# wsakobe/CylinderTag

Measured on AMD Instinct MI355X. Metric: frames/sec detect() 1920x1080, higher is better.
Workload: dtype u8; 1 GPU; synthetic 1920x1080 random-stripe frames, 4096 per step over 1 GPU(s), 4 planted CTag_2f12c markers each, detect(img,5,true,5), inputs resident in HBM; frames_per_gpu=4096, chunk=4096, parallelism=frames sharded, dp1, gather=none (1 GPU)

## Files before the change

cylindertag_amd/csrc/ctag_api.hip:

```cpp
#include <hip/hip_runtime.h>

#include <algorithm>
#include <climits>
#include <cmath>
#include <cstdio>
#include <cstdlib>
#include <cstring>
#include <fstream>
#include <map>
#include <mutex>
#include <new>
#include <string>
#include <type_traits>
#include <vector>

#include "../../include/ctag.h"
#include "ctag_internal.h"

using namespace ctag;

#define HIP_TRY(expr)                                                                                   \
    do {                                                                                                \
        hipError_t e__ = (expr);                                                                        \
        if (e__ != hipSuccess) {                                                                        \
// ... 123 lines not shown
    struct {
        void* p = nullptr;
        void (*free_fn)(void*) = nullptr;
    } state[kNumSiblingStates];
};

namespace ctag {
void** handle_state_slot(ctag_handle* h, SiblingState which, void (*free_fn)(void*)) {
    h->state[which].free_fn = free_fn;
    return &h->state[which].p;
}
bool handle_timing(const ctag_handle* h) { return h->timing; }
int handle_device(const ctag_handle* h) { return h->device; }
int handle_dict_cols(const ctag_handle* h) { return h->dict_cols; }
void handle_view(const ctag_handle* h, HandleView* out) {
    out->device = h->device;
    out->ws = h->last_ws && h->last_ws->base ? h->last_ws : nullptr;
    out->last_chunk_frames = h->last_chunk_frames;
    out->keep_pre = h->keep_pre;
    out->dict = h->dict.data();
    out->dict_rows = h->dict_rows;
    out->dict_cols = h->dict_cols;
    out->fused = h->last_plan.fused;
    out->frames = h->last_frames;
    out->row_stride = h->last_row_stride;
    out->frame_stride = h->last_frame_stride;
    out->stream = h->stream;
    out->gray = h->last_was_bgr ? h->d_gray.p : nullptr;
    out->gray_row_stride = h->gray_row_stride;
    out->gray_frame_stride = h->gray_frame_stride;
}
}

static const char* kStageNames[CTAG_NUM_STAGES] = {"decimate",  "threshold_ccl", "seam_merge", "resolve", "candidates", "quad_pack", "quad_edges", "quad_edges_big",
                                                    "line_sort", "welsch",        "quad_final", "features", "edge_refine", "markers"};

static FrameGeom make_geom(int rows, int cols, int tw, double area_max_fraction = 0.01) {
    FrameGeom g{};
    g.rows = rows;
    g.cols = cols;
    g.hrows = rows / 2;
    g.hcols = cols / 2;
    g.hp = (g.hcols + 63) & ~63;
    g.lp = (g.hcols + 63) & ~63;
    g.tw = tw;
    g.trows = g.hrows / tw + (g.hrows % tw != 0 ? 1 : 0);
// ... 96 lines not shown
    put(W.ymax, pool);
    put(W.key, pool);
    put(W.pool_tile, pool);
    put(W.member_head, pool);
    put(W.member_next, pool);
    put(W.ncand, F * 4);
    put(W.nroots, F * 4);
    put(W.cand, F * CC * sizeof(Candidate));
    put(W.quads, F * CC * sizeof(QuadOut));
    put(W.line_count, F * 4);
    put(W.clp_used, F * 4);
    put(W.line_long, F * 4);
    put(W.cl_pool, F * (size_t)W.cl_cap * 4 + 16);
    put(W.line_desc, F * LC * sizeof(LineDesc));
    put(W.line_sorted, F * LC * 4);
    put(W.line_fit, F * LC * 16);
    put(W.cand_aux, F * CC * sizeof(CandAux));
    put(W.npacks, F * 8);
    put(W.packs, F * CC * 4);
    put(W.pack_order, F * CC * 4);
    put(W.npacks2, F * 8);
    put(W.packs2, F * CC * 4);
    put(W.pack_order2, F * CC * 4);
    put(W.welsch_rs, std::min<size_t>(F, kLatencyFrames) * kLatLines * 20 * 6 * 4);
    put(W.quad_derived, F * kQuadStride * 48);
    put(W.quad_index, F * kQuadStride * 4);
    put(W.nquads, F * 4);
    put(W.nfeat, F * 4);
    put(W.status, F * 4);
    put(W.feat0, F * CTAG_MAX_FEATURES * sizeof(FeatureDev));
    put(W.feat1, F * CTAG_MAX_FEATURES * sizeof(FeatureDev));
    put(W.feat2, F * CTAG_MAX_FEATURES * sizeof(FeatureDev));
    put(W.premarkers, F * sizeof(ctag_frame_result));
    put(W.frame_long, F * 4);
    put(W.rz_xofs, (size_t)g.hcols * 4);
    put(W.rz_alpha, (size_t)g.hcols * 8);
    put(W.rz_yofs, (size_t)g.hrows * 4);
    put(W.rz_beta, (size_t)g.hrows * 8);
    return off;
}

static int ensure_workspace(ctag_handle* h, ctag_handle::WsSlot& S, int rows, int cols, int tw, int frames, bool big, bool need_n0) {
    auto refresh = [&](Workspace& W) {
        const Caps c = make_caps(make_geom(rows, cols, tw, h->params.area_max_fraction), h->params, big);
        W.g = make_geom(rows, cols, tw, h->params.area_max_fraction);
        W.g.pool_cap = c.pool_cap;
// ... 1025 lines not shown
```

cylindertag_amd/csrc/ctag_internal.h:

```cpp
#pragma once
#include <hip/hip_runtime.h>
#include <stddef.h>
#include <stdint.h>

#include <vector>

#include "../../include/ctag_types.h"

struct ctag_handle;
struct ctag_camera;
struct ctag_pose_rec;
struct ctag_rig_pose_rec;
struct ctag_mv_pose_rec;
struct ctag_camera_set;

namespace ctag {
template <class T>
struct DevBuf {
    T* p = nullptr;
    size_t cap = 0;
    DevBuf() = default;
    DevBuf(const DevBuf&) = delete;
    DevBuf& operator=(const DevBuf&) = delete;
    ~DevBuf() { release(); }
// ... 155 lines not shown
    int32_t* member_next = nullptr;
    int32_t* ncand = nullptr;
    int32_t* nroots = nullptr;
    int cand_cap = 0;
    int line_cap = 0;
    uint32_t cl_cap = 0;
    bool big = false;
    Candidate* cand = nullptr;
    QuadOut* quads = nullptr;
    int32_t* line_count = nullptr;
    int32_t* clp_used = nullptr;
    uint32_t* cl_pool = nullptr;
    LineDesc* line_desc = nullptr;
    int32_t* line_sorted = nullptr;
    int32_t* line_long = nullptr;
    float* line_fit = nullptr;
    CandAux* cand_aux = nullptr;
    int32_t* npacks = nullptr;
    uint32_t* packs = nullptr;
    uint32_t* pack_order = nullptr;
    int32_t* npacks2 = nullptr;
    uint32_t* packs2 = nullptr;
    uint32_t* pack_order2 = nullptr;
    float* welsch_rs = nullptr;
    const uint8_t* pick_table = nullptr;
    const uint16_t* pick_table16 = nullptr;
    hipStream_t aux_stream = nullptr;
    hipEvent_t ev_fork = nullptr, ev_join = nullptr;
    KParams kp{};
    void* quad_derived = nullptr;
    int32_t* quad_index = nullptr;
    int32_t* nquads = nullptr;
    int32_t* nfeat = nullptr;
    int32_t* status = nullptr;
    FeatureDev* feat0 = nullptr;
    FeatureDev* feat1 = nullptr;
    FeatureDev* feat2 = nullptr;
    ctag_frame_result* premarkers = nullptr;
    double* refine_n0 = nullptr;
    int32_t* frame_long = nullptr;
    int32_t* rz_xofs = nullptr;
    int16_t* rz_alpha = nullptr;
    int32_t* rz_yofs = nullptr;
    int16_t* rz_beta = nullptr;
    void* base = nullptr;
    size_t bytes = 0;
// ... 104 lines not shown
void build_pick_table(uint8_t* table, uint16_t* table16);


enum SiblingState { kPoseState, kDrawState, kRigState, kGatherState, kMvState, kCovState, kFitState, kRigFitState, kCamFitState, kIntrFitState, kNumSiblingStates };
void** handle_state_slot(struct ::ctag_handle* h, SiblingState which, void (*free_fn)(void*));
int model_to_device(struct ::ctag_model* m, int device);
int rigs_to_device(struct ::ctag_rigs* r, int device);
bool camera_ok(const struct ::ctag_camera* c);
bool handle_timing(const struct ::ctag_handle* h);
int handle_finish_pending(struct ::ctag_handle* h);
bool handle_pending_state(struct ::ctag_handle* h, const int32_t** count_dev, uint64_t* gen);
void handle_pending_clean(struct ::ctag_handle* h, uint64_t gen);
int handle_device(const struct ::ctag_handle* h);
int handle_dict_cols(const struct ::ctag_handle* h);

struct HandleView {
    int device;
    const Workspace* ws;
    int last_chunk_frames;
    bool keep_pre;
    const int32_t* dict;
    int dict_rows, dict_cols;
    bool fused;
    const uint8_t* frames;
    ptrdiff_t row_stride, frame_stride;
    hipStream_t stream;
    const uint8_t* gray;
    ptrdiff_t gray_row_stride, gray_frame_stride;
};
void handle_view(const struct ::ctag_handle* h, HandleView* out);
int mfit_probe_system(struct ::ctag_handle* h, const ctag_frame_result* results, int n_frames, const struct ::ctag_pose_rec* poses, int n_poses,
                      const struct ::ctag_model* model, const struct ::ctag_camera* camera, int model_index, double lambda, int min_obs, int pass_records,
                      double* S, double* g, double* delta, int32_t* held, int32_t* bad_pivot);
int mfit_record_grid();
int mfit_pass_records();
int rfit_probe_system(struct ::ctag_handle* h, const ctag_frame_result* results, int n_frames, const struct ::ctag_rig_pose_rec* recs,
                      const struct ::ctag_model* model, const struct ::ctag_rigs* rigs, const struct ::ctag_camera* camera, int rig, double lambda,
                      int pass_records, double* S, double* g, double* delta, int32_t* n_unknowns, int32_t* bad_pivot);
int cfit_probe_system(struct ::ctag_handle* h, const ctag_frame_result* results, int n_frames, const struct ::ctag_mv_pose_rec* recs,
                      const struct ::ctag_model* model, const struct ::ctag_rigs* rigs, const struct ::ctag_camera_set* cams, int anchor, double lambda,
                      int pass_records, double* S, double* g, double* delta, int32_t* n_unknowns, int32_t* bad_pivot);
int ifit_probe_system(struct ::ctag_handle* h, const ctag_frame_result* results, int n_frames, const struct ::ctag_rig_pose_rec* recs,
                      const struct ::ctag_model* model, const struct ::ctag_rigs* rigs, const struct ::ctag_camera* camera, uint32_t free_mask, int tie_focal,
                      double lambda, int pass_records, double* S, double* g, double* delta, int32_t* n_free, int32_t* bad_pivot);
int ifit_probe_poses(struct ::ctag_handle* h, const ctag_frame_result* results, int n_frames, const struct ::ctag_rig_pose_rec* recs,
                     const struct ::ctag_model* model, const struct ::ctag_rigs* rigs, const struct ::ctag_camera* camera, struct ::ctag_rig_pose_rec* out,
// ... 11 lines not shown
```

cylindertag_amd/csrc/k_quad.hip:

```cpp
#include "ctag_internal.h"
#include "ctag_math.h"
#include "ctag_wave.h"
#include <cstdio>
#include <type_traits>
#include <cstdlib>

namespace ctag {

struct QuadPtrs {
    const uint16_t* labels;
    const int32_t* tile_base;
    const int32_t* root_of;
    const int32_t* ncand;
    const Candidate* cand;
    QuadOut* quads;
    uint32_t* frame_flags;
    int32_t* line_count;
    int32_t* clp_used;
    uint32_t* cl_pool;
    LineDesc* line_desc;
    int32_t* line_sorted;
    int32_t* line_long;
    float* line_fit;
    CandAux* cand_aux;
    const uint8_t* pick_table;
    const uint16_t* pick_table16;
    const int32_t* pool_tile;
    const int32_t* member_head;
    const int32_t* member_next;
    int32_t* npacks;
    uint32_t* packs;
    uint32_t* pack_order;
    int32_t* npacks2;
    uint32_t* packs2;
    uint32_t* pack_order2;
    unsigned long long* stamps;
    float thr_line, thr_expand, rac;
    int c2_far, c2_near;
    int cand_cap, line_cap;
    uint32_t cl_cap;
    float expand_eps;
    const uint64_t* mask;
    int mask_words;
};
static QuadPtrs quad_ptrs(const ChunkPlan& pl, const Workspace& ws, unsigned long long* stamps) {
    QuadPtrs P{};
    P.labels = ws.labels, P.tile_base = ws.tile_base, P.root_of = ws.root_of, P.ncand = ws.ncand, P.cand = ws.cand, P.quads = ws.quads, P.frame_flags = ws.frame_flags;
    P.line_count = ws.line_count, P.clp_used = ws.clp_used, P.cl_pool = ws.cl_pool, P.line_desc = ws.line_desc, P.line_sorted = ws.line_sorted, P.line_long = ws.line_long;
    P.line_fit = ws.line_fit, P.cand_aux = ws.cand_aux, P.pick_table = ws.pick_table, P.pick_table16 = ws.pick_table16;
    P.pool_tile = ws.pool_tile, P.member_head = ws.member_head, P.member_next = ws.member_next;
    P.npacks = ws.npacks, P.packs = ws.packs, P.pack_order = ws.pack_order, P.stamps = stamps;
    P.npacks2 = ws.npacks2, P.packs2 = ws.packs2, P.pack_order2 = ws.pack_order2;
    P.thr_line = ws.kp.thr_line, P.thr_expand = ws.kp.thr_expand, P.rac = ws.kp.rac, P.c2_far = ws.kp.c2_far, P.c2_near = ws.kp.c2_near, P.expand_eps = ws.kp.expand_eps;
    P.cand_cap = ws.cand_cap, P.line_cap = ws.line_cap, P.cl_cap = ws.cl_cap;
    P.mask = pl.fused ? reinterpret_cast<const uint64_t*>(ws.half) : nullptr, P.mask_words = ws.g.hcols >> 6;
    return P;
}

__device__ __forceinline__ uint32_t pack_xy(int x, int y) { return (uint32_t)x | ((uint32_t)y << 16); }
__device__ __forceinline__ int ux(uint32_t p) { return (int)(p & 0xffffu); }
__device__ __forceinline__ int uy(uint32_t p) { return (int)(p >> 16); }

__device__ __forceinline__ void moments_to_line(double x, double y, double x2, double y2, double xy, double w, float* line) {
    const ctm::Recip64 W = ctm::recip64(w);
    x = ctm::div64(x, W);
    y = ctm::div64(y, W);
    x2 = ctm::div64(x2, W);
    y2 = ctm::div64(y2, W);
    xy = ctm::div64(xy, W);
    const double dx2 = x2 - x * x, dy2 = y2 - y * y, dxy = xy - x * y;
    const float t = (float)ctm::atan2_64(2 * dxy, dx2 - dy2) / 2;
    double sn, cs;
    ctm::sincos64(t, &sn, &cs);
    line[0] = (float)cs;
    line[1] = (float)sn;
// ... 218 lines not shown
    restart_store(res, rstride, line, err);
}

#ifndef CTAG_PACK_WORDS
#define CTAG_PACK_WORDS 5120
#endif
#ifndef CTAG_PACK_WAVES
#define CTAG_PACK_WAVES 2
#endif
constexpr int kPackWords = CTAG_PACK_WORDS;
#ifndef CTAG_PACK_WAVES_P2
#define CTAG_PACK_WAVES_P2 4
#endif
constexpr int kPackWordsSmall = 2560, kPackWavesSmall = 4, kPackWavesSmallP2 = CTAG_PACK_WAVES_P2;
constexpr int kUnwind = 8;
constexpr int kWaveWords = 8192;
constexpr int kWaveWordsMax = 36864;
__host__ __device__ __forceinline__ int pack_points(int w, int h) { return min(2 * (w + h), w * h) + 1; }
__host__ __device__ __forceinline__ int pack_need(int w, int h) {
    const int C = pack_points(w, h);
    return ((w + 1) & ~1) + 2 * h + 2 * C + 4;
}
__host__ __device__ __forceinline__ int need2(int n) { return 2 * ((n + 1) & ~1); }
constexpr int kScanWords = 2048;
__host__ __device__ __forceinline__ int scan_need(int w, int h) { return w + 3 * h + 4; }
constexpr int kMaskScanWords = 512, kMaskScanWordsLarge = 2048;
__host__ __device__ __forceinline__ int mask_scan_need(int w, int h) { return h * ((w + 31) / 32 + 1); }
__host__ __device__ __forceinline__ bool pack_big(int x_min, int w, int h, int big_points, int pack_words, int scan_words = 0) {
    (void)x_min;
    return pack_need(w, h) > pack_words || pack_points(w, h) > big_points || (scan_words > 0 && scan_need(w, h) > scan_words) ||
           (scan_words < 0 && mask_scan_need(w, h) > -scan_words);
}

struct CornerPre {
    float x, y, dis, ang;
};

__device__ __forceinline__ int pack_rank_sort(const int* s_key, uint16_t* s_ord, int n, int tid, int nt) {
    int neg = 0;
    for (int i = tid; i < n; i += nt) {
        const int ki = s_key[i];
        int rank = 0;
        for (int j = 0; j < n; j++) {
            const int kj = s_key[j];
            rank += (kj > ki || (kj == ki && j < i)) ? 1 : 0;
        }
// ... 137 lines not shown
    uint32_t* order2 = P.pack_order2 + (size_t)frame * P.cand_cap;
    uint32_t* packs2 = P.packs2 + (size_t)frame * P.cand_cap;
    auto key_of = [&](int r) {
        const CandAux a = aux[order[r]];
        return (a.line0 >= 0 && a.n_boundary > 0) ? a.n_boundary : -1;
    };
    int nel, np;
    if (npk > kLdsCand) {
        nel = pack_counting_sort(s_key, order2, npk, tid, nt, key_of, [&](int r) { return order[r]; });
        np = build_packs(packs2, nel, max_per_pack, pack_words, tid, [&](int r) { return need2(aux[order2[r]].n_boundary); });
    } else {
        for (int r = tid; r < npk; r += nt) s_key[r] = key_of(r);
        if (tid == 0) s_key[kLdsCand] = 0;
        __syncthreads();
        if (const int neg = pack_rank_sort(s_key, s_ord, npk, tid, nt)) atomicAdd(&s_key[kLdsCand], neg);
        __syncthreads();
        nel = npk - s_key[kLdsCand];
        for (int i = tid; i < nel; i += nt) order2[i] = order[s_ord[i]];
        np = build_packs(packs2, nel, max_per_pack, pack_words, tid, [&](int r) { return need2(s_key[s_ord[r]]); });
    }
    if (tid == 0) {
        P.npacks2[2 * frame] = np;
        P.npacks2[2 * frame + 1] = nel;
    }
}


#ifndef CTAG_EXPAND_INLINE
#define CTAG_EXPAND_INLINE __forceinline__
#endif
struct ALine {
    double c, s, x, y;
    bool ok;
};
__device__ __forceinline__ ALine approx_line(long long sx, long long sy, long long sxx, long long syy, long long sxy, int cnt, double k2lim) {
    const double n = (double)cnt, fx = (double)sx, fy = (double)sy;
    const double rn = __builtin_amdgcn_rcp(n);
    const double A = ((double)sxx * n - fx * fx) - ((double)syy * n - fy * fy);
    const double B = 2.0 * ((double)sxy * n - fx * fy);
    const double h2 = A * A + B * B;
    const double rh = __builtin_amdgcn_rsq(h2);
    const double u = ctm::fabs64(A) * rh;
    const double p = 0.5 + 0.5 * u;
    const double rp = __builtin_amdgcn_rsq(p);
    const double big = p * rp, small = (0.5 * ctm::fabs64(B) * rh) * rp;
    const bool bneg = B < 0.0;
// ... 368 lines not shown
                aux->line0 = p0;
                aux->acx = 0.f;
                aux->acy = 0.f;
                aux->n_boundary = 0;
            }
        }
    }
}

template <int SG, int WORDS, int WAVES, bool DYN, bool REFPRM, int PHASE = 0, bool PRESCAN = false>
__global__ __launch_bounds__(64) __attribute__((amdgpu_waves_per_eu(WAVES, WAVES))) void k_quad_edges_packed(QuadPtrs P, FrameGeom g, int nframes, int tier_lo) {
    static_assert(PHASE != 3 || (SG == 64 && !PRESCAN), "the scan-only build is a whole-wave build");
    static_assert(!PRESCAN || (SG == 8 && PHASE != 2), "PRESCAN: a packed build that would otherwise scan");
    const float k_thr_line = REFPRM ? 1.8f : P.thr_line, k_thr_expand = REFPRM ? 1.2f : P.thr_expand;
    const int k_c2_far = REFPRM ? 2 : P.c2_far, k_c2_near = REFPRM ? 1 : P.c2_near;
    static_assert(SG == 8 || SG == 64, "8 lanes per component (packs) or the whole wave (oversize components)");
    __shared__ uint32_t s_static[DYN ? 1 : WORDS];
    extern __shared__ uint32_t s_dynamic[];
    uint32_t* const s_mem = DYN ? s_dynamic : s_static;
    const int frame = blockIdx.x;
    if (frame >= nframes) return;
    const int lane = threadIdx.x, sub = lane / SG, sl = lane % SG, lane0 = lane - sl;
    const int nc = min(P.ncand[frame], P.cand_cap);
    const int npk = PHASE == 3 ? nc - P.npacks[2 * frame + 1]
                  : PHASE == 2 ? P.npacks2[2 * frame]
                               : P.npacks[2 * frame + (SG == 8 ? 0 : 1)];
    static_assert(PHASE != 2 || SG == 8, "the second kernel is a packed build");
    const uint32_t* __restrict__ pack_list = (PHASE == 2 ? P.packs2 : P.packs) + (size_t)frame * P.cand_cap;
    const uint32_t* __restrict__ pack_ord = (PHASE == 2 ? P.pack_order2 : P.pack_order) + (size_t)frame * P.cand_cap;
    const uint16_t* __restrict__ limg = P.labels + ((size_t)frame * g.hrows) * g.lp;
    const int32_t* __restrict__ tbase = P.tile_base + (size_t)frame * g.tiles_x * g.tiles_y;
    const int32_t* __restrict__ rootof = P.root_of + (size_t)frame * g.pool_cap;

    unsigned long long t_prev = 0;
    auto stamp = [&](int phase) {
        if (P.stamps) {
            const unsigned long long t = __builtin_amdgcn_s_memtime();
            if (phase >= 0 && lane == 0) atomicAdd(&P.stamps[phase + (SG == 64 ? 8 : 0)], t - t_prev);
            t_prev = t;
        }
    };
    for (int pk = blockIdx.y; pk < npk; pk += gridDim.y) {
        __syncthreads();
        stamp(-1);
        int first, cnt;
        if constexpr (SG == 8) {
            const uint32_t pw = pack_list[pk];
            first = (int)(pw & 0xffffffu);
            cnt = (int)(pw >> 24);
        } else if constexpr (PHASE == 3) {
            first = pk;
            cnt = 1;
        } else {
            first = nc - npk + pk;
            cnt = 1;
        }
        const bool act = sub < cnt;
        const int ci = (int)pack_ord[first + (act ? sub : 0)];
        const Candidate cd = P.cand[(size_t)frame * P.cand_cap + ci];
        CandAux* aux = P.cand_aux + (size_t)frame * P.cand_cap + ci;
        const int x_min = cd.x_min, y_min = cd.y_min;
        const int w = cd.x_max - cd.x_min + 1, h = cd.y_max - cd.y_min + 1;
        const int C = pack_points(w, h);
        int nb2 = 0;
        if constexpr (PHASE == 2) nb2 = aux->n_boundary;
        const int need = act ? (PHASE == 3 ? scan_need(w, h) : PHASE == 2 ? need2(nb2) : pack_need(w, h)) : 0;
        int off = 0;
#pragma unroll
        for (int k = 0; k < 64 / SG; k++) {
            const int v = __shfl(need, k * SG);
            if (k < sub) off += v;
        }
        if (!act) continue;
        if constexpr (SG == 64 && PHASE != 3) {
            if (need <= tier_lo) continue;
            if (need > WORDS) {
                if (tier_lo > 0 && sl == 0) {
                    atomicOr(&P.frame_flags[frame], CTAG_FLAG_POOL_OVERFLOW);
                    aux->line0 = -1;
                    aux->acx = 0.f;
                    aux->acy = 0.f;
                    aux->n_boundary = 0;
                }
                continue;
            }
        }
        uint32_t* mem = s_mem + off;
        uint32_t* tb = mem;
        uint32_t* lr = tb + w + 2;
        uint32_t* bufA = PHASE == 2 ? mem + (need >> 1) : lr + h + 2;
        uint32_t* bufB = PHASE == 2 ? mem : bufA + (PHASE == 3 ? h : C);
        uint32_t* lef = bufA;
        uint32_t* rig = bufB;
        const int sgshift = sub * SG;

        int n = 0, n_boundary = 0, p0 = 0;
        float acx = 0.f, acy = 0.f;
        if constexpr (PHASE != 2 && !PRESCAN) {
        stamp(6);
#ifndef CTAG_KEYS_LARGE
#define CTAG_KEYS_LARGE 16
#endif
#ifndef CTAG_KEYS_SMALL
#define CTAG_KEYS_SMALL 8
#endif
        constexpr int kMaxKeys = (SG == 8 && WORDS > kPackWordsSmall) ? CTAG_KEYS_LARGE : CTAG_KEYS_SMALL;
        uint32_t mykey[kMaxKeys];
        bool many = false;
        {
            const int32_t* ptile = P.pool_tile + (size_t)frame * g.pool_cap;
            const int32_t* mnext = P.member_next + (size_t)frame * g.pool_cap;
            int e = cd.root;
            bool first_e = true;
#pragma unroll
// ... 482 lines not shown
                }
                continue;
            }
            uint32_t* slot = P.cl_pool + (size_t)frame * P.cl_cap + p0;
            for (int x = sl; x < w + 2; x += SG) slot[x] = tb[x];
            for (int y = sl; y < h + 2; y += SG) slot[w + 2 + y] = lr[y];
            if (sl == 0) {
                aux->line0 = p0;
                aux->acx = 0.f;
                aux->acy = 0.f;
                aux->n_boundary = 0;
            }
            continue;
        }
        if constexpr (PHASE != 2) {
        if constexpr (PRESCAN) {
            p0 = aux->line0;
            if (p0 < 0) continue;
            const uint32_t* slot = P.cl_pool + (size_t)frame * P.cl_cap + p0;
            for (int x = sl; x < w + 2; x += SG) tb[x] = slot[x];
            for (int y = sl; y < h + 2; y += SG) lr[y] = slot[w + 2 + y];
            wave_fence();
        }
        int ntotal = 0;
        for (int x = sl; x < w; x += SG) {
            const uint32_t t = tb[x + 1];
            if (t) ntotal += 1 + ((t & 0xffffu) != (t >> 16) ? 1 : 0);
        }
        for (int y = sl; y < h; y += SG) {
            const uint32_t v = lr[y + 1];
            if (v) {
                const uint32_t ky = (uint32_t)(y + 2), xl = (v & 0xffffu) - 2u, xr = (v >> 16) - 2u;
                const uint32_t tl = tb[xl + 1], tr = tb[xr + 1];
                if ((tl & 0xffffu) != ky && (tl >> 16) != ky) ntotal++;
                if (xr != xl && (tr & 0xffffu) != ky && (tr >> 16) != ky) ntotal++;
            }
        }
        ntotal = sg_sum<SG>(ntotal);
        stamp(0);
        n = 0;
        {
            const int jd = sl & 7;
            const int dxl = (int)((0x01A9u >> (2 * jd)) & 3u) - 1, dyl = (int)((0x1A90u >> (2 * jd)) & 3u) - 1;
            int sp = 0;
            int fx = 0, fy = 0, j0 = 0;
            {
                const uint32_t c0 = tb[1];
                if (c0 == 0u) {
                    sp = -1;
                } else {
                    fy = (int)(c0 & 0xffffu) - 2;
                    n = 1;
                }
            }
            wave_fence();
            if (sp >= 0 && sl == 0) {
                bufA[0] = pack_xy(x_min, fy + y_min);
                uint32_t c = tb[1];
                if ((c >> 16) == (uint32_t)(fy + 2)) c &= 0xffffu;
                c &= 0xffff0000u;
                tb[1] = c;
// ... 66 lines not shown
                        }
                    }
                }
            } else {
                while (sp >= 0 && n < ntotal) {
                    const int nx = fx + dxl, ny = fy + dyl;
                    const uint32_t c = tb[nx + 1], r = lr[ny + 1];
                    const uint32_t ky = (uint32_t)(ny + 2), kx = (uint32_t)(nx + 2);
                    const bool hit = sl < 8 && sl >= j0 && ((c & 0xffffu) == ky || (c >> 16) == ky || (r & 0xffffu) == kx || (r >> 16) == kx);
                    const unsigned m = (unsigned)((__ballot(hit) >> sgshift) & 0xffull);
                    if (!m) {
                        sp--;
                        if (sp >= 0) {
                            const uint32_t f = bufB[sp];
                            fx = (int)(f & 0x3fff);
                            fy = (int)((f >> 14) & 0x3fff);
                            j0 = (int)(f >> 28);
                        }
                        continue;
                    }
                    const int j = __ffs(m) - 1;
                    const int hx = fx + ((int)((0x01A9u >> (2 * j)) & 3u) - 1), hy = fy + ((int)((0x1A90u >> (2 * j)) & 3u) - 1);
                    if (sl == j) {
                        if (n < C) bufA[n] = pack_xy(hx + x_min, hy + y_min);
                        uint32_t c2 = c, r2 = r;
                        if ((c2 & 0xffffu) == ky) c2 &= 0xffff0000u;
                        if ((c2 >> 16) == ky) c2 &= 0xffffu;
                        if ((r2 & 0xffffu) == kx) r2 &= 0xffff0000u;
                        if ((r2 >> 16) == kx) r2 &= 0xffffu;
                        tb[nx + 1] = c2;
                        lr[ny + 1] = r2;
                        if (sp <= C) bufB[sp] = (uint32_t)hx | ((uint32_t)hy << 14) | ((uint32_t)(j + 1) << 28);
                    }
                    wave_fence();
                    n++;
                    fx = hx;
                    fy = hy;
                    if (sp + 1 <= C) {
                        sp++;
                        j0 = 0;
                    } else {
                        j0 = j + 1;
                    }
                }
            }
            n = min(n, C);
        }
        n_boundary = n;
        if (n == 0) {
            if (sl == 0) {
                aux->line0 = -1;
                aux->acx = 0.f;
                aux->acy = 0.f;
                aux->n_boundary = 0;
            }
            continue;
        }
        wave_fence();
        stamp(1);
        {
            unsigned long long sx = 0, sy = 0;
            for (int k = sl; k < n; k += SG) {
                sx += (unsigned)ux(bufA[k]);
                sy += (unsigned)uy(bufA[k]);
            }
            sx = (unsigned long long)sg_sum<SG>((long long)sx);
            sy = (unsigned long long)sg_sum<SG>((long long)sy);
            acx = (float)(1.0 * (long long)sx / (double)(unsigned long long)n);
            acy = (float)(1.0 * (long long)sy / (double)(unsigned long long)n);
// ... 879 lines not shown
    out->valid = valid;
#pragma unroll
    for (int j = 0; j < 4; j++) {
        out->c[2 * j] = valid ? bc[j].x : 0.f;
        out->c[2 * j + 1] = valid ? bc[j].y : 0.f;
    }
}

#ifndef CTAG_SCAN_WAVES
#define CTAG_SCAN_WAVES 4
#endif
template <bool REF>
static void launch_quad_edges(const ChunkPlan& pl, const QuadPtrs& P, const FrameGeom& g, hipStream_t s, hipStream_t sb, hipStream_t s_max, hipEvent_t mid) {
    const int nframes = pl.nframes;
    const dim3 grid(nframes, pl.pack_gx);
    if (pl.all_wave) {
    } else if (pl.prescan) {
        if (pl.mask_scan)
            if (pl.small_cfg) hipLaunchKernelGGL((k_silhouette_mask<4, 32, kMaskScanWords>), dim3(nframes, pl.mscan_gx), dim3(64), 0, s, P, g, nframes);
            else hipLaunchKernelGGL((k_silhouette_mask<8, 64, kMaskScanWordsLarge>), dim3(nframes, 2 * pl.mscan_gx), dim3(64), 0, s, P, g, nframes);
        else
            hipLaunchKernelGGL((k_quad_edges_packed<64, kScanWords, CTAG_SCAN_WAVES, false, true, 3>), dim3(nframes, pl.scan_gx), dim3(64), 0, s, P, g, nframes, 0);
        if (pl.small_cfg) {
            hipLaunchKernelGGL((k_quad_edges_packed<8, kPackWordsSmall, kPackWavesSmall, false, REF, 1, true>), grid, dim3(64), 0, s, P, g, nframes, 0);
            hipLaunchKernelGGL(k_repack, dim3(nframes), dim3(64), 0, s, P, nframes, pl.pack_max, kPackWordsSmall);
            hipLaunchKernelGGL((k_quad_edges_packed<8, kPackWordsSmall, kPackWavesSmallP2, false, REF, 2>), grid, dim3(64), 0, s, P, g, nframes, 0);
        } else {
            hipLaunchKernelGGL((k_quad_edges_packed<8, kPackWords, CTAG_PACK_WAVES, false, REF, 0, true>), grid, dim3(64), 0, s, P, g, nframes, 0);
        }
    } else if (pl.small_cfg) {
        hipLaunchKernelGGL((k_quad_edges_packed<8, kPackWordsSmall, kPackWavesSmall, false, REF, 1>), grid, dim3(64), 0, s, P, g, nframes, 0);
        hipLaunchKernelGGL(k_repack, dim3(nframes), dim3(64), 0, s, P, nframes, pl.pack_max, kPackWordsSmall);
        hipLaunchKernelGGL((k_quad_edges_packed<8, kPackWordsSmall, kPackWavesSmallP2, false, REF, 2>), grid, dim3(64), 0, s, P, g, nframes, 0);
    } else {
        hipLaunchKernelGGL((k_quad_edges_packed<8, kPackWords, CTAG_PACK_WAVES, false, REF>), grid, dim3(64), 0, s, P, g, nframes, 0);
    }
    if (mid) (void)hipEventRecord(mid, s);
    ensure_dynamic_lds(reinterpret_cast<const void*>(&k_quad_edges_packed<64, kWaveWordsMax, 1, true, REF>), kWaveWordsMax * 4);
    hipLaunchKernelGGL((k_quad_edges_packed<64, kWaveWords, 1, false, REF>), dim3(nframes, pl.big_cols), dim3(64), 0, sb, P, g, nframes, 0);
    hipLaunchKernelGGL((k_quad_edges_packed<64, kWaveWordsMax, 1, true, REF>), dim3(nframes, pl.big_max_gx), dim3(64), kWaveWordsMax * 4, s_max, P, g, nframes, kWaveWords);
}

hipError_t launch_line_fits(const ChunkPlan& pl, const Workspace& ws, hipStream_t s, unsigned long long* stamps, hipEvent_t ev_sorted) {
    const int nframes = pl.nframes;
    const QuadPtrs P = quad_ptrs(pl, ws, stamps);
    hipLaunchKernelGGL(k_line_sort, dim3(nframes), dim3(kLineSortThreads), 0, s, P, nframes);
// ... 105 lines not shown
```

include/ctag_testkit.h:

```cpp
#ifndef CTAG_TESTKIT_H
#define CTAG_TESTKIT_H
#include <stddef.h>
#include <stdint.h>

#include "ctag.h"
#include "ctag_pose.h"

#ifdef __cplusplus
extern "C" {
#endif

#define CTAG_DBG_HALF 1
#define CTAG_DBG_LABELS 2
#define CTAG_DBG_CANDIDATES 3
#define CTAG_DBG_CAND_QUADS 4
#define CTAG_DBG_FEATURES0 5
#define CTAG_DBG_FEATURES1 6
#define CTAG_DBG_FEATURES2 7
#define CTAG_DBG_PREMARKERS 8
#define CTAG_DBG_GRAY 9
#define CTAG_DBG_MASK 11
#define CTAG_DBG_LINES 10
#define CTAG_DBG_LINE_POINTS 12
#define CTAG_DBG_LINE_FITS 13
#define CTAG_DBG_PACKS 14
long ctag_debug_fetch(ctag_handle* h, int frame, int what, void* dst, size_t capacity_elems);

int ctag_math_probe(ctag_handle* h, int op, int n, const double* a, const double* b, double* out);

int ctag_testkit_exp32_k0_sweep(uint32_t first_bits, uint32_t last_bits, uint32_t step, uint64_t* counts, uint32_t* first_bad);

int ctag_testkit_unpack_gathered(ctag_handle* h, const void* gathered_dev, int n_total, int world, uint64_t width,
                                 ctag_frame_result* out_dev);

int ctag_testkit_stall_stream(ctag_handle* h, int milliseconds);

typedef struct ctag_synth_truth {
    int32_t n_markers;
    int32_t dict_row[8];
    float strip_len[8];
    float corners[8][8];
} ctag_synth_truth;
int ctag_synth_frames_device(ctag_handle* h, uint8_t* frames_dev, int first_frame, int n, int rows, int cols,
                             ptrdiff_t row_stride, ptrdiff_t frame_stride, uint64_t seed, int markers_per_frame);
int ctag_synth_frame_host(const int32_t* state, int dict_rows, int dict_cols, uint8_t* frame, int frame_index, int rows,
                          int cols, ptrdiff_t row_stride, uint64_t seed, int markers_per_frame, ctag_synth_truth* truth);
int ctag_synth_layout_truth(const int32_t* state, int dict_rows, int dict_cols, int frame_index, int rows, int cols, uint64_t seed,
                            int markers_per_frame, ctag_synth_truth* truth);
// ... 55 lines not shown
```

testkit/__init__.py:

```python
import ctypes as C
import os
import subprocess

import numpy as np

import cylindertag_amd as ca
from cylindertag_amd import capi
from cylindertag_amd.capi import CtagError, Model

_HERE = os.path.dirname(os.path.abspath(__file__))
_LIB = os.environ.get("CTAG_TESTKIT_LIB") or os.path.join(_HERE, "_build", "libctag_testkit.so")

TRUTH3D_DT = np.dtype([("n_markers", "<i4"), ("dict_row", "<i4", (8,)), ("_pad", "<i4", (1,)), ("R", "<f8", (8, 9)), ("t", "<f8", (8, 3)),
                       ("radius", "<f8", (8,))])
TRUTH_DT = np.dtype([("n_markers", "<i4"), ("dict_row", "<i4", (8,)), ("strip_len", "<f4", (8,)),
                     ("corners", "<f4", (8, 8))])
DBG_HALF, DBG_LABELS, DBG_CANDIDATES, DBG_CAND_QUADS, DBG_FEATURES0, DBG_FEATURES1, DBG_FEATURES2, DBG_PREMARKERS, DBG_GRAY, DBG_LINES, DBG_MASK, DBG_LINE_POINTS, DBG_LINE_FITS, DBG_PACKS = range(1, 15)
SYNTH_SEED = 0x4354616753594E00

EXPORTS = ["ctag_debug_fetch", "ctag_math_probe", "ctag_testkit_exp32_k0_sweep", "ctag_testkit_unpack_gathered", "ctag_testkit_stall_stream", "ctag_synth_frames_device", "ctag_synth_frame_host",
           "ctag_synth_layout_truth", "ctag_synth3d_frames_device", "ctag_synth3d_frame_host", "ctag_synth3d_model",
           "ctag_testkit_dense_edge_probe", "ctag_testkit_plan", "ctag_testkit_welsch_fit", "ctag_testkit_welsch_limits",
           "ctag_testkit_model_fit_system", "ctag_testkit_model_fit_limits", "ctag_testkit_rig_fit_system", "ctag_testkit_rig_fit_limits",
           "ctag_testkit_camera_fit_system", "ctag_testkit_camera_fit_limits",
           "ctag_testkit_intrinsics_fit_system", "ctag_testkit_intrinsics_fit_poses", "ctag_testkit_intrinsics_fit_limits"]
PLAN_FIELDS = ("fused", "bgr_direct", "zero_first", "dec_zero_kernel", "dec_zero_list", "dec", "dec_xblocks", "dec_yblocks", "dec_band_rows", "dec_bands",
               "ccl", "latency", "small_cfg", "refprm", "mask_scan", "prescan", "all_wave", "fork", "pack_max", "big_points", "pack_gx", "scan_gx",
               "mscan_gx", "big_cols", "big_max_gx", "welsch_gs", "welsch_gx", "refine", "refine_gx", "refine_sums_gx")
DEC_FORMS = ("mask", "mask_bands", "general", "wide", "banded135", "banded", "unaligned")
CCL_FORMS = ("mask", "tw5", "any")
WELSCH_LIMITS = ("kWShort", "kWCap", "kWRes", "kWPts", "kWPtsU", "kPickN", "kPickN2", "kWE", "kWT", "kLatLines", "kLatPoints", "kLatChunk", "kLdsLines",
                 "kLatencyFrames", "kLatRankBlocks", "kLineSortBuckets")
REFINE_FORMS = ("none", "one", "split_large", "split_looping", "split")
MATH_EXP32_NONPOS, MATH_EXP32_NONPOS_K0 = 15, 17


def lib_path():
    return _LIB


# ... 200 lines not shown
            raise CtagError(st, "ctag_synth_frames_device")

    def synth3d_frames_device(self, frames_ptr, first, n, rows, cols, row_stride, frame_stride, K, seed=SYNTH_SEED, markers=4):
        K = np.asarray(K, np.float64)
        st = self.T.ctag_synth3d_frames_device(self.h, frames_ptr, first, n, rows, cols, row_stride, frame_stride, seed, markers,
                                               K[0, 0], K[1, 1], K[0, 2], K[1, 2])
        if st != 0:
            raise CtagError(st, "ctag_synth3d_frames_device")

    def stall_stream(self, milliseconds):
        st = self.T.ctag_testkit_stall_stream(self.h, int(milliseconds))
        if st != 0:
            raise CtagError(st, "ctag_testkit_stall_stream")

    def unpack_gathered(self, gathered_ptr, n_total, world, width, out_ptr):
        self._gcheck(self.T.ctag_testkit_unpack_gathered(self.h, gathered_ptr, n_total, world, width, out_ptr), "ctag_testkit_unpack_gathered")

    def debug(self, frame, what):
        n = self.T.ctag_debug_fetch(self.h, frame, what, None, 0)
        if n < 0:
            raise CtagError(-1, "ctag_debug_fetch(%d)" % what)
        if what in (DBG_HALF, DBG_GRAY, DBG_MASK):
            a = np.zeros(n, np.uint8)
        elif what in (DBG_LABELS, DBG_CANDIDATES, DBG_LINES, DBG_LINE_POINTS, DBG_PACKS):
            a = np.zeros(n, np.int32)
        elif what == DBG_PREMARKERS:
            a = np.zeros(1, ca.RESULT_DT)
        else:
            a = np.zeros(n, np.float32)
        if n:
            got = self.T.ctag_debug_fetch(self.h, frame, what, a.ctypes.data, max(n, 1))
            if got < 0:
                raise CtagError(-2, "ctag_debug_fetch(%d)" % what)
        if what in (DBG_CANDIDATES, DBG_CAND_QUADS):
            return a.reshape(-1, 8)
        if what in (DBG_FEATURES0, DBG_FEATURES1, DBG_FEATURES2):
            return a.reshape(-1, 19)
        if what == DBG_PREMARKERS:
            return a[0]
        if what == DBG_LINE_POINTS:
            return a.reshape(-1, 2)
        if what == DBG_LINE_FITS:
            return a.reshape(-1, 4)
        return a

    def welsch_fit(self, frames, latency=0, welsch_gx=0, welsch_gs=0, tail_at_pool_end=False):
        clusters = [np.asarray(c, np.int32).reshape(-1, 2) for f in frames for c in f]
# ... 109 lines not shown
```

testkit/ctag_testkit.hip:

```cpp
#include <hip/hip_runtime.h>

#include <algorithm>
#include <cstring>
#include <vector>

#include "../include/ctag_testkit.h"
#include "../cylindertag_amd/csrc/ctag_internal.h"
#include "../cylindertag_amd/csrc/ctag_math.h"
#include "ctag_synth.h"

using namespace ctag;

#define TK_TRY(expr)                              \
    do {                                          \
        if ((expr) != hipSuccess) return CTAG_ERR_HIP; \
    } while (0)

namespace {

__global__ void k_math_probe(int op, int n, const double* a, const double* b, double* out) {
    const int i = blockIdx.x * blockDim.x + threadIdx.x;
    if (i >= n) return;
    const double x = a[i], y = b[i];
    double r = 0;
// ... 369 lines not shown
        case CTAG_DBG_PACKS: {
            int32_t hd[5] = {0, 0, 0, 0, 0};
            if (!d2h(&hd[0], W.ncand + frame, 4) || !d2h(&hd[1], W.npacks + 2 * frame, 8) || !d2h(&hd[3], W.npacks2 + 2 * frame, 8)) return -2;
            hd[0] = std::min(hd[0], W.cand_cap);
            const size_t nc = (size_t)hd[0], np1 = (size_t)hd[1], np2 = (size_t)hd[3], nel = (size_t)hd[4];
            if (hd[1] < 0 || hd[3] < 0 || hd[4] < 0 || np1 > nc || np2 > nc || nel > nc) return -2;
            const size_t total = 5 + np1 + np2 + nc + nel + nc;
            if (dst && cap >= total) {
                int32_t* o = static_cast<int32_t*>(dst);
                std::memcpy(o, hd, sizeof(hd));
                o += 5;
                const size_t fo = (size_t)frame * W.cand_cap;
                if (np1 && !d2h(o, W.packs + fo, np1 * 4)) return -2;
                o += np1;
                if (np2 && !d2h(o, W.packs2 + fo, np2 * 4)) return -2;
                o += np2;
                if (nc && !d2h(o, W.pack_order + fo, nc * 4)) return -2;
                o += nc;
                if (nel && !d2h(o, W.pack_order2 + fo, nel * 4)) return -2;
                o += nel;
                std::vector<CandAux> a(std::max<size_t>(nc, 1));
                if (nc && !d2h(a.data(), W.cand_aux + fo, nc * sizeof(CandAux))) return -2;
                for (size_t i = 0; i < nc; i++) o[i] = a[i].n_boundary;
            }
            return (long)total;
        }
        case CTAG_DBG_PREMARKERS: {
            if (!v.keep_pre) return -1;
            if (dst && cap >= 1) {
                if (!d2h(dst, W.premarkers + frame, sizeof(ctag_frame_result))) return -2;
            }
            return 1;
        }
        default: return -1;
    }
}

int ctag_math_probe(ctag_handle* h, int op, int n, const double* a, const double* b, double* out) {
    if (!h || n < 0 || !a || !out) return CTAG_ERR_ARG;
    if (n == 0) return CTAG_OK;
    HandleView v{};
    handle_view(h, &v);
    TK_TRY(hipSetDevice(v.device));
    hipStream_t s = static_cast<hipStream_t>(ctag_stream(h));
    double *da = nullptr, *db = nullptr, *dout = nullptr;
    int rc = CTAG_OK;
// ... 297 lines not shown
```

Measured before the change: 271,800 frames/s.

## Prescan silhouette point counts to repack phase-1 quad edge builds tighter

Adds a k_prepack kernel that counts the silhouette boundary points of each candidate ahead of time, then sorts and repacks candidates using an exact LDS need based on that count instead of the worst-case perimeter. The phase-1 packed edge kernel reads the precomputed count and the new pack lists, so it drops its own count loop and can fit more candidates per LDS pack. This trades an extra kernel launch and extra global buffers for better LDS packing and fewer or smaller packs in the edge trace stage.

```diff
diff --git a/cylindertag_amd/csrc/ctag_api.hip b/cylindertag_amd/csrc/ctag_api.hip
--- a/cylindertag_amd/csrc/ctag_api.hip
+++ b/cylindertag_amd/csrc/ctag_api.hip
@@ -169,6 +169,7 @@
     out->dict_rows = h->dict_rows;
     out->dict_cols = h->dict_cols;
     out->fused = h->last_plan.fused;
+    out->packs1 = !h->last_plan.all_wave && h->last_plan.prescan && h->last_plan.small_cfg;
     out->frames = h->last_frames;
     out->row_stride = h->last_row_stride;
     out->frame_stride = h->last_frame_stride;
@@ -311,6 +312,10 @@
     put(W.npacks2, F * 8);
     put(W.packs2, F * CC * 4);
     put(W.pack_order2, F * CC * 4);
+    put(W.npacks1, F * 8);
+    put(W.packs1, F * CC * 4);
+    put(W.pack_order1, F * CC * 4);
+    put(W.ntotal1, F * CC * 4);
     put(W.welsch_rs, std::min<size_t>(F, kLatencyFrames) * kLatLines * 20 * 6 * 4);
     put(W.quad_derived, F * kQuadStride * 48);
     put(W.quad_index, F * kQuadStride * 4);
diff --git a/cylindertag_amd/csrc/ctag_internal.h b/cylindertag_amd/csrc/ctag_internal.h
--- a/cylindertag_amd/csrc/ctag_internal.h
+++ b/cylindertag_amd/csrc/ctag_internal.h
@@ -201,6 +201,10 @@
     int32_t* npacks2 = nullptr;
     uint32_t* packs2 = nullptr;
     uint32_t* pack_order2 = nullptr;
+    int32_t* npacks1 = nullptr;
+    uint32_t* packs1 = nullptr;
+    uint32_t* pack_order1 = nullptr;
+    int32_t* ntotal1 = nullptr;
     float* welsch_rs = nullptr;
     const uint8_t* pick_table = nullptr;
     const uint16_t* pick_table16 = nullptr;
@@ -351,6 +355,7 @@
     const int32_t* dict;
     int dict_rows, dict_cols;
     bool fused;
+    bool packs1;
     const uint8_t* frames;
     ptrdiff_t row_stride, frame_stride;
     hipStream_t stream;
diff --git a/cylindertag_amd/csrc/k_quad.hip b/cylindertag_amd/csrc/k_quad.hip
--- a/cylindertag_amd/csrc/k_quad.hip
+++ b/cylindertag_amd/csrc/k_quad.hip
@@ -34,6 +34,10 @@
     int32_t* npacks2;
     uint32_t* packs2;
     uint32_t* pack_order2;
+    int32_t* npacks1;
+    uint32_t* packs1;
+    uint32_t* pack_order1;
+    int32_t* ntotal1;
     unsigned long long* stamps;
     float thr_line, thr_expand, rac;
     int c2_far, c2_near;
@@ -51,6 +55,7 @@
     P.pool_tile = ws.pool_tile, P.member_head = ws.member_head, P.member_next = ws.member_next;
     P.npacks = ws.npacks, P.packs = ws.packs, P.pack_order = ws.pack_order, P.stamps = stamps;
     P.npacks2 = ws.npacks2, P.packs2 = ws.packs2, P.pack_order2 = ws.pack_order2;
+    P.npacks1 = ws.npacks1, P.packs1 = ws.packs1, P.pack_order1 = ws.pack_order1, P.ntotal1 = ws.ntotal1;
     P.thr_line = ws.kp.thr_line, P.thr_expand = ws.kp.thr_expand, P.rac = ws.kp.rac, P.c2_far = ws.kp.c2_far, P.c2_near = ws.kp.c2_near, P.expand_eps = ws.kp.expand_eps;
     P.cand_cap = ws.cand_cap, P.line_cap = ws.line_cap, P.cl_cap = ws.cl_cap;
     P.mask = pl.fused ? reinterpret_cast<const uint64_t*>(ws.half) : nullptr, P.mask_words = ws.g.hcols >> 6;
@@ -315,6 +320,7 @@
     return ((w + 1) & ~1) + 2 * h + 2 * C + 4;
 }
 __host__ __device__ __forceinline__ int need2(int n) { return 2 * ((n + 1) & ~1); }
+__host__ __device__ __forceinline__ int need1(int w, int h, int nt) { return (w + h + 2 * nt + 6) & ~1; }
 constexpr int kScanWords = 2048;
 __host__ __device__ __forceinline__ int scan_need(int w, int h) { return w + 3 * h + 4; }
 constexpr int kMaskScanWords = 512, kMaskScanWordsLarge = 2048;
@@ -498,6 +504,95 @@
     if (tid == 0) {
         P.npacks2[2 * frame] = np;
         P.npacks2[2 * frame + 1] = nel;
+    }
+}
+
+template <int SG, int U = 1>
+__device__ __forceinline__ int silhouette_points(const uint32_t* tb, const uint32_t* lr, int w, int h, int sl) {
+    int nt = 0;
+    for (int x0 = sl; x0 < w; x0 += SG * U) {
+        uint32_t t[U];
+#pragma unroll
+        for (int u = 0; u < U; u++) t[u] = x0 + SG * u < w ? tb[x0 + SG * u + 1] : 0u;
+#pragma unroll
+        for (int u = 0; u < U; u++)
+            if (t[u]) nt += 1 + ((t[u] & 0xffffu) != (t[u] >> 16) ? 1 : 0);
+    }
+    for (int y0 = sl; y0 < h; y0 += SG * U) {
+        uint32_t v[U], tl[U], tr[U];
+#pragma unroll
+        for (int u = 0; u < U; u++) v[u] = y0 + SG * u < h ? lr[y0 + SG * u + 1] : 0u;
+#pragma unroll
+        for (int u = 0; u < U; u++) {
+            tl[u] = v[u] ? tb[min((v[u] & 0xffffu) - 2u, (uint32_t)(w - 1)) + 1] : 0u;
+            tr[u] = v[u] ? tb[min((v[u] >> 16) - 2u, (uint32_t)(w - 1)) + 1] : 0u;
+        }
+#pragma unroll
+        for (int u = 0; u < U; u++)
+            if (v[u]) {
+                const uint32_t ky = (uint32_t)(y0 + SG * u + 2);
+                if ((tl[u] & 0xffffu) != ky && (tl[u] >> 16) != ky) nt++;
+                if ((v[u] >> 16) != (v[u] & 0xffffu) && (tr[u] & 0xffffu) != ky && (tr[u] >> 16) != ky) nt++;
+            }
+    }
+    return sg_sum<SG>(nt);
+}
+
+constexpr int kPrepackThreads = 256;
+__global__ __launch_bounds__(kPrepackThreads) void k_prepack(QuadPtrs P, int nframes, int max_per_pack, int pack_words) {
+    __shared__ int s_key[kLdsCand + 2];
+    __shared__ int s_need[kLdsCand];
+    __shared__ uint16_t s_ord[kLdsCand];
+    const int frame = blockIdx.x;
+    if (frame >= nframes) return;
+    const int tid = threadIdx.x, nt = blockDim.x, sub = tid >> 3, sl = tid & 7;
+    const int nc = min(P.ncand[frame], P.cand_cap);
+    const int npk = max(nc - P.npacks[2 * frame + 1], 0);
+    const Candidate* cand = P.cand + (size_t)frame * P.cand_cap;
+    const CandAux* aux = P.cand_aux + (size_t)frame * P.cand_cap;
+    const uint32_t* order = P.pack_order + (size_t)frame * P.cand_cap;
+    uint32_t* order1 = P.pack_order1 + (size_t)frame * P.cand_cap;
+    uint32_t* packs1 = P.packs1 + (size_t)frame * P.cand_cap;
+    int32_t* ntot = P.ntotal1 + (size_t)frame * P.cand_cap;
+    const bool in_lds = npk <= kLdsCand;
+    for (int r0 = 0; r0 < npk; r0 += nt >> 3) {
+        const int r = r0 + sub;
+        const bool act = r < npk;
+        const int ci = (int)order[act ? r : 0];
+        const Candidate c = cand[ci];
+        const int p0 = aux[ci].line0;
+        const bool has = act && p0 >= 0;
+        const int w = has ? c.x_max - c.x_min + 1 : 0, h = has ? c.y_max - c.y_min + 1 : 0;
+        const uint32_t* slot = P.cl_pool + (size_t)frame * P.cl_cap + (has ? p0 : 0);
+        const int cnt = silhouette_points<8, 4>(slot, slot + w + 2, w, h, sl);
+        if (act && sl == 0) {
+            ntot[ci] = has ? cnt : -1;
+            if (in_lds) s_key[r] = has ? cnt : -1, s_need[r] = need1(w, h, cnt);
+        }
+    }
+    __syncthreads();
+    auto need_of_cand = [&](int ci) {
+        const Candidate c = cand[ci];
+        return need1(c.x_max - c.x_min + 1, c.y_max - c.y_min + 1, ntot[ci]);
+    };
+    int nel, np;
+    if (!in_lds) {
+        nel = pack_counting_sort(s_key, order1, npk, tid, nt, [&](int r) { return (int)ntot[order[r]]; }, [&](int r) { return order[r]; });
+        if (tid >= 64) return;
+        np = build_packs(packs1, nel, max_per_pack, pack_words, tid, [&](int r) { return need_of_cand((int)order1[r]); });
+    } else {
+        if (tid == 0) s_key[kLdsCand] = 0;
+        __syncthreads();
+        if (const int neg = pack_rank_sort(s_key, s_ord, npk, tid, nt)) atomicAdd(&s_key[kLdsCand], neg);
+        __syncthreads();
+        nel = npk - s_key[kLdsCand];
+        for (int i = tid; i < nel; i += nt) order1[i] = order[s_ord[i]];
+        if (tid >= 64) return;
+        np = build_packs(packs1, nel, max_per_pack, pack_words, tid, [&](int r) { return s_need[s_ord[r]]; });
+    }
+    if (tid == 0) {
+        P.npacks1[2 * frame] = np;
+        P.npacks1[2 * frame + 1] = nel;
     }
 }
 
@@ -912,12 +1007,14 @@
     if (frame >= nframes) return;
     const int lane = threadIdx.x, sub = lane / SG, sl = lane % SG, lane0 = lane - sl;
     const int nc = min(P.ncand[frame], P.cand_cap);
+    constexpr bool PACKS1 = PRESCAN && PHASE == 1;
     const int npk = PHASE == 3 ? nc - P.npacks[2 * frame + 1]
                   : PHASE == 2 ? P.npacks2[2 * frame]
-                               : P.npacks[2 * frame + (SG == 8 ? 0 : 1)];
+                  : PACKS1 ? P.npacks1[2 * frame]
+                           : P.npacks[2 * frame + (SG == 8 ? 0 : 1)];
     static_assert(PHASE != 2 || SG == 8, "the second kernel is a packed build");
-    const uint32_t* __restrict__ pack_list = (PHASE == 2 ? P.packs2 : P.packs) + (size_t)frame * P.cand_cap;
-    const uint32_t* __restrict__ pack_ord = (PHASE == 2 ? P.pack_order2 : P.pack_order) + (size_t)frame * P.cand_cap;
+    const uint32_t* __restrict__ pack_list = (PHASE == 2 ? P.packs2 : PACKS1 ? P.packs1 : P.packs) + (size_t)frame * P.cand_cap;
+    const uint32_t* __restrict__ pack_ord = (PHASE == 2 ? P.pack_order2 : PACKS1 ? P.pack_order1 : P.pack_order) + (size_t)frame * P.cand_cap;
     const uint16_t* __restrict__ limg = P.labels + ((size_t)frame * g.hrows) * g.lp;
     const int32_t* __restrict__ tbase = P.tile_base + (size_t)frame * g.tiles_x * g.tiles_y;
     const int32_t* __restrict__ rootof = P.root_of + (size_t)frame * g.pool_cap;
@@ -954,7 +1051,9 @@
         const int C = pack_points(w, h);
         int nb2 = 0;
         if constexpr (PHASE == 2) nb2 = aux->n_boundary;
-        const int need = act ? (PHASE == 3 ? scan_need(w, h) : PHASE == 2 ? need2(nb2) : pack_need(w, h)) : 0;
+        int nt1 = 0;
+        if constexpr (PACKS1) nt1 = P.ntotal1[(size_t)frame * P.cand_cap + ci];
+        const int need = act ? (PHASE == 3 ? scan_need(w, h) : PHASE == 2 ? need2(nb2) : PACKS1 ? need1(w, h, nt1) : pack_need(w, h)) : 0;
         int off = 0;
 #pragma unroll
         for (int k = 0; k < 64 / SG; k++) {
@@ -978,8 +1077,9 @@
         uint32_t* mem = s_mem + off;
         uint32_t* tb = mem;
         uint32_t* lr = tb + w + 2;
+        const int cap = PACKS1 ? nt1 : C;
         uint32_t* bufA = PHASE == 2 ? mem + (need >> 1) : lr + h + 2;
-        uint32_t* bufB = PHASE == 2 ? mem : bufA + (PHASE == 3 ? h : C);
+        uint32_t* bufB = PHASE == 2 ? mem : bufA + (PHASE == 3 ? h : cap);
         uint32_t* lef = bufA;
         uint32_t* rig = bufB;
         const int sgshift = sub * SG;
@@ -1508,21 +1608,7 @@
             for (int y = sl; y < h + 2; y += SG) lr[y] = slot[w + 2 + y];
             wave_fence();
         }
-        int ntotal = 0;
-        for (int x = sl; x < w; x += SG) {
-            const uint32_t t = tb[x + 1];
-            if (t) ntotal += 1 + ((t & 0xffffu) != (t >> 16) ? 1 : 0);
-        }
-        for (int y = sl; y < h; y += SG) {
-            const uint32_t v = lr[y + 1];
-            if (v) {
-                const uint32_t ky = (uint32_t)(y + 2), xl = (v & 0xffffu) - 2u, xr = (v >> 16) - 2u;
-                const uint32_t tl = tb[xl + 1], tr = tb[xr + 1];
-                if ((tl & 0xffffu) != ky && (tl >> 16) != ky) ntotal++;
-                if (xr != xl && (tr & 0xffffu) != ky && (tr >> 16) != ky) ntotal++;
-            }
-        }
-        ntotal = sg_sum<SG>(ntotal);
+        const int ntotal = PACKS1 ? nt1 : silhouette_points<SG>(tb, lr, w, h, sl);
         stamp(0);
         n = 0;
         {
@@ -1635,7 +1721,7 @@
                     const int j = __ffs(m) - 1;
                     const int hx = fx + ((int)((0x01A9u >> (2 * j)) & 3u) - 1), hy = fy + ((int)((0x1A90u >> (2 * j)) & 3u) - 1);
                     if (sl == j) {
-                        if (n < C) bufA[n] = pack_xy(hx + x_min, hy + y_min);
+                        if (n < cap) bufA[n] = pack_xy(hx + x_min, hy + y_min);
                         uint32_t c2 = c, r2 = r;
                         if ((c2 & 0xffffu) == ky) c2 &= 0xffff0000u;
                         if ((c2 >> 16) == ky) c2 &= 0xffffu;
@@ -1643,13 +1729,13 @@
                         if ((r2 >> 16) == kx) r2 &= 0xffffu;
                         tb[nx + 1] = c2;
                         lr[ny + 1] = r2;
-                        if (sp <= C) bufB[sp] = (uint32_t)hx | ((uint32_t)hy << 14) | ((uint32_t)(j + 1) << 28);
+                        if (sp <= cap) bufB[sp] = (uint32_t)hx | ((uint32_t)hy << 14) | ((uint32_t)(j + 1) << 28);
                     }
                     wave_fence();
                     n++;
                     fx = hx;
                     fy = hy;
-                    if (sp + 1 <= C) {
+                    if (sp + 1 <= cap) {
                         sp++;
                         j0 = 0;
                     } else {
@@ -1657,7 +1743,7 @@
                     }
                 }
             }
-            n = min(n, C);
+            n = min(n, cap);
         }
         n_boundary = n;
         if (n == 0) {
@@ -2583,6 +2669,7 @@
         else
             hipLaunchKernelGGL((k_quad_edges_packed<64, kScanWords, CTAG_SCAN_WAVES, false, true, 3>), dim3(nframes, pl.scan_gx), dim3(64), 0, s, P, g, nframes, 0);
         if (pl.small_cfg) {
+            hipLaunchKernelGGL(k_prepack, dim3(nframes), dim3(kPrepackThreads), 0, s, P, nframes, pl.pack_max, kPackWordsSmall);
             hipLaunchKernelGGL((k_quad_edges_packed<8, kPackWordsSmall, kPackWavesSmall, false, REF, 1, true>), grid, dim3(64), 0, s, P, g, nframes, 0);
             hipLaunchKernelGGL(k_repack, dim3(nframes), dim3(64), 0, s, P, nframes, pl.pack_max, kPackWordsSmall);
             hipLaunchKernelGGL((k_quad_edges_packed<8, kPackWordsSmall, kPackWavesSmallP2, false, REF, 2>), grid, dim3(64), 0, s, P, g, nframes, 0);
diff --git a/include/ctag_testkit.h b/include/ctag_testkit.h
--- a/include/ctag_testkit.h
+++ b/include/ctag_testkit.h
@@ -24,6 +24,7 @@
 #define CTAG_DBG_LINE_POINTS 12
 #define CTAG_DBG_LINE_FITS 13
 #define CTAG_DBG_PACKS 14
+#define CTAG_DBG_PACKS1 15
 long ctag_debug_fetch(ctag_handle* h, int frame, int what, void* dst, size_t capacity_elems);
 
 int ctag_math_probe(ctag_handle* h, int op, int n, const double* a, const double* b, double* out);
diff --git a/testkit/__init__.py b/testkit/__init__.py
--- a/testkit/__init__.py
+++ b/testkit/__init__.py
@@ -15,7 +15,7 @@
                        ("radius", "<f8", (8,))])
 TRUTH_DT = np.dtype([("n_markers", "<i4"), ("dict_row", "<i4", (8,)), ("strip_len", "<f4", (8,)),
                      ("corners", "<f4", (8, 8))])
-DBG_HALF, DBG_LABELS, DBG_CANDIDATES, DBG_CAND_QUADS, DBG_FEATURES0, DBG_FEATURES1, DBG_FEATURES2, DBG_PREMARKERS, DBG_GRAY, DBG_LINES, DBG_MASK, DBG_LINE_POINTS, DBG_LINE_FITS, DBG_PACKS = range(1, 15)
+DBG_HALF, DBG_LABELS, DBG_CANDIDATES, DBG_CAND_QUADS, DBG_FEATURES0, DBG_FEATURES1, DBG_FEATURES2, DBG_PREMARKERS, DBG_GRAY, DBG_LINES, DBG_MASK, DBG_LINE_POINTS, DBG_LINE_FITS, DBG_PACKS, DBG_PACKS1 = range(1, 16)
 SYNTH_SEED = 0x4354616753594E00
 
 EXPORTS = ["ctag_debug_fetch", "ctag_math_probe", "ctag_testkit_exp32_k0_sweep", "ctag_testkit_unpack_gathered", "ctag_testkit_stall_stream", "ctag_synth_frames_device", "ctag_synth_frame_host",
@@ -262,7 +262,7 @@
             raise CtagError(-1, "ctag_debug_fetch(%d)" % what)
         if what in (DBG_HALF, DBG_GRAY, DBG_MASK):
             a = np.zeros(n, np.uint8)
-        elif what in (DBG_LABELS, DBG_CANDIDATES, DBG_LINES, DBG_LINE_POINTS, DBG_PACKS):
+        elif what in (DBG_LABELS, DBG_CANDIDATES, DBG_LINES, DBG_LINE_POINTS, DBG_PACKS, DBG_PACKS1):
             a = np.zeros(n, np.int32)
         elif what == DBG_PREMARKERS:
             a = np.zeros(1, ca.RESULT_DT)
diff --git a/testkit/ctag_testkit.hip b/testkit/ctag_testkit.hip
--- a/testkit/ctag_testkit.hip
+++ b/testkit/ctag_testkit.hip
@@ -415,6 +415,34 @@
                 std::vector<CandAux> a(std::max<size_t>(nc, 1));
                 if (nc && !d2h(a.data(), W.cand_aux + fo, nc * sizeof(CandAux))) return -2;
                 for (size_t i = 0; i < nc; i++) o[i] = a[i].n_boundary;
+            }
+            return (long)total;
+        }
+        case CTAG_DBG_PACKS1: {
+            int32_t hd[4] = {0, v.packs1 ? 1 : 0, 0, 0};
+            if (!d2h(&hd[0], W.ncand + frame, 4)) return -2;
+            hd[0] = std::min(hd[0], W.cand_cap);
+            if (v.packs1 && !d2h(&hd[2], W.npacks1 + 2 * frame, 8)) return -2;
+            const size_t nc = (size_t)hd[0], np = (size_t)hd[2], nel = (size_t)hd[3];
+            if (hd[2] < 0 || hd[3] < 0 || np > nc || nel > nc) return -2;
+            if (!v.packs1) {
+                if (dst && cap >= 4) std::memcpy(dst, hd, sizeof(hd));
+                return 4;
+            }
+            const size_t total = 4 + np + nel + nc;
+            if (dst && cap >= total) {
+                int32_t* o = static_cast<int32_t*>(dst);
+                std::memcpy(o, hd, sizeof(hd));
+                o += 4;
+                const size_t fo = (size_t)frame * W.cand_cap;
+                if (np && !d2h(o, W.packs1 + fo, np * 4)) return -2;
+                o += np;
+                if (nel && !d2h(o, W.pack_order1 + fo, nel * 4)) return -2;
+                std::vector<int32_t> nt(std::max<size_t>(nc, 1));
+                if (nc && !d2h(nt.data(), W.ntotal1 + fo, nc * 4)) return -2;
+                for (size_t i = 0; i < nc; i++) o[nel + i] = -1;
+                for (size_t i = 0; i < nel; i++)
+                    if (o[i] >= 0 && (size_t)o[i] < nc) o[nel + o[i]] = nt[o[i]];
             }
             return (long)total;
         }
```

Result: faster. 280,600 frames/s, median of 6 (+3.2%).
